# Gwzwpxz/HDSDP

Hardware: AMD Instinct MI355X
Metric: IPM iterations/sec (Schur build+factor+solve), n=2000 m=2000 dense SDP (higher is better)
Workload: dtype f64

## Files before the change

hdsdp_amd/csrc/chol.hip:

```cpp
#include "hdm_common.h"
#include "chol.h"
#include "sweep128.h"
#include <algorithm>
#include <atomic>
#include <cstring>

#define NB 128

#define PB 32
#define LDW 98
__device__ __forceinline__ double hdm_readlane_f64(double v, int lane) {
    int lo = __double2loint(v), hi = __double2hiint(v);
    lo = __builtin_amdgcn_readlane(lo, lane);
    hi = __builtin_amdgcn_readlane(hi, lane);
    return __hiloint2double(hi, lo);
}

typedef double hdm_c4 __attribute__((ext_vector_type(4)));

template <int NT>
__device__ __forceinline__ void hdm_lds_mm(double *pc, int crs, int ccs, const double *pa, int ars, int acs, const double *pb,
                                           int brs, int bcs, int M, int N, int K, double alpha, int accumulate, int k_by_row,
                                           int lower_only, int wave, int lane, double *gout, long gld) {
    const int l15 = lane & 15, lq = lane >> 4;
    const int mt = M >> 4, nt = (N >> 4) / NT, units = mt * nt;
    for (int u = wave; u < units; u += 4) {
        const int ti = u / nt, tj = (u % nt) * NT;
        if (lower_only && tj > ti) continue;
        hdm_c4 acc[NT];
#pragma unroll
        for (int q = 0; q < NT; ++q) acc[q] = (hdm_c4){0.0, 0.0, 0.0, 0.0};
        const int kend = k_by_row ? min(K, (ti + 1) * 16) : K;
        const double *qa = pa + (ti * 16 + l15) * ars + lq * acs;
        const double *qb = pb + lq * brs + (tj * 16 + l15) * bcs;
        for (int k0 = 0; k0 < kend; k0 += 4) {
            const double av = qa[k0 * acs];
#pragma unroll
            for (int q = 0; q < NT; ++q) acc[q] = __builtin_amdgcn_mfma_f64_16x16x4f64(qb[k0 * brs + q * 16 * bcs], av, acc[q], 0, 0, 0);
        }
#pragma unroll
        for (int q = 0; q < NT; ++q)
#pragma unroll
            for (int r = 0; r < 4; ++r) {
                const int m = ti * 16 + l15, n = (tj + q) * 16 + lq + 4 * r;
                double *c = pc + m * crs + n * ccs;
                const double v = (accumulate ? *c : 0.0) + alpha * acc[q][r];
                *c = v;
                if (gout) gout[m + (long) n * gld] = v;
            }
    }
}

__global__ __launch_bounds__(256) void hdm_potrf_diag_kernel(double *__restrict__ A, long ld, double *__restrict__ Dinv,
                                                              int *__restrict__ info, int col0) {
    extern __shared__ __attribute__((aligned(16))) double sm[];
    double *a = sm;
    double *w = sm + NB * NB;
    const int tid = threadIdx.x;
    for (int e0 = tid; e0 < NB * NB; e0 += 256 * 16) {
        double v[16];
#pragma unroll
        for (int q = 0; q < 16; ++q) {
            const int e = e0 + q * 256;
            v[q] = A[(e & (NB - 1)) + (long) (e >> 7) * ld];
        }
#pragma unroll
        for (int q = 0; q < 16; ++q) {
            const int e = e0 + q * 256;
            a[e] = ((e & (NB - 1)) >= (e >> 7)) ? v[q] : 0.0;
        }
    }
    __syncthreads();

    for (int p = 0; p < NB / PB; ++p) {
        const int c0 = p * PB;
        if (tid < 64) {
            const int l = tid & 31;
            double *blk = a + c0 + c0 * NB;
            double row[PB], rinv[PB];
#pragma unroll
            for (int k = 0; k < PB; ++k) row[k] = blk[l + k * NB];
            int bad = 0;
#pragma unroll
            for (int j = 0; j < PB; ++j) {
                double d = hdm_readlane_f64(row[j], j);
                if (!(d > 0.0)) {
                    if (!bad) bad = j + 1;
                    d = 1.0;
                }
                const double piv = sqrt(d);
                double ri = 1.0 / piv;
                asm volatile("" : "+v"(ri));
                rinv[j] = ri;
                row[j] = (l == j) ? piv : row[j] * ri;
#pragma unroll
                for (int k = j + 1; k < PB; ++k) row[k] -= row[j] * hdm_readlane_f64(row[j], k);
                __builtin_amdgcn_sched_barrier(0);
            }
            if (bad && tid == 0) atomicCAS(info, 0, col0 + c0 + bad);
            if (tid < PB) {
#pragma unroll
                for (int k = 0; k < PB; ++k)
                    if (k <= l) A[(c0 + l) + (long) (c0 + k) * ld] = row[k];
            }
#pragma unroll
            for (int k = 0; k < PB; ++k) asm volatile("" : "+v"(row[k]));
            double x[PB];
#pragma unroll
            for (int i = 0; i < PB; ++i) {
                double sacc = (l == i) ? 1.0 : 0.0;
#pragma unroll
                for (int k = 0; k < i; ++k) sacc -= hdm_readlane_f64(row[k], i) * x[k];
                x[i] = (l <= i) ? sacc * rinv[i] : 0.0;
                __builtin_amdgcn_sched_barrier(0);
            }
            if (tid < PB) {
#pragma unroll
                for (int i = 0; i < PB; ++i) blk[i + l * NB] = x[i];
            }
        }
        __syncthreads();
        const int t0 = c0 + PB, nr = NB - t0;
        if (nr <= 0) break;
        const int wave = tid >> 6, lane = tid & 63;
        hdm_lds_mm<2>(a + t0 + c0 * NB, 1, NB, a + t0 + c0 * NB, 1, NB, a + c0 + c0 * NB, NB, 1, nr, PB, PB, 1.0, 0, 0, 0, wave,
                      lane, A + t0 + (long) c0 * ld, ld);
        __syncthreads();
        hdm_lds_mm<1>(a + t0 + t0 * NB, 1, NB, a + t0 + c0 * NB, 1, NB, a + t0 + c0 * NB, NB, 1, nr, nr, PB, -1.0, 1, 0, 1, wave,
                      lane, nullptr, 0);
        __syncthreads();
    }
    {
        const int wave = tid >> 6, lane = tid & 63;
        for (int j = NB / PB - 2; j >= 0; --j) {
            const int c0 = j * PB, r0 = c0 + PB, nr = NB - r0;
            hdm_lds_mm<2>(w, 1, LDW, a + r0 + c0 * NB, 1, NB, a + c0 + c0 * NB, 1, NB, nr, PB, PB, 1.0, 0, 0, 0, wave, lane,
                          nullptr, 0);
            __syncthreads();
            hdm_lds_mm<2>(a + r0 + c0 * NB, 1, NB, a + r0 + r0 * NB, 1, NB, w, 1, LDW, nr, PB, nr, -1.0, 0, 1, 0, wave, lane,
                          nullptr, 0);
            __syncthreads();
        }
    }
    for (int e = tid; e < NB * NB; e += 256) Dinv[e] = a[e];
}

#define DIAG_SWEEP_LDS_DOUBLES (SMALL_P * (SMALL_P + 1) + 2 * SMALL_P)
template <bool SIGNED = false>
__device__ __forceinline__ void hdm_potrf_diag_sweep_body(double *__restrict__ A, long ld, double *__restrict__ Dinv, int *__restrict__ info,
                                                          int col0, int nv, double *__restrict__ sgn_out = nullptr,
                                                          int *__restrict__ nneg_out = nullptr) {
    extern __shared__ __attribute__((aligned(16))) double sm[];
    double *img = sm;
    double *rsv = sm + SMALL_P * (SMALL_P + 1);
    constexpr int ldi = SMALL_P + 1;
    const int tid = threadIdx.x, ty = tid >> 5, tx = tid & 31;
    const int ei = tid & (SMALL_P - 1), ej0 = tid >> 7;
#pragma unroll 8
    for (int j = ej0; j < SMALL_P; j += SM_T / SMALL_P) img[ei + j * ldi] = (ei >= j) ? A[ei + (long) j * ld] : 0.0;
    __syncthreads();
    double a[SM_NR][SM_NC], rr[SM_NR][SM_NC];
#pragma unroll
    for (int r = 0; r < SM_NR; ++r)
#pragma unroll
        for (int c = 0; c < SM_NC; ++c) a[r][c] = img[(ty + 16 * r) + (tx + 32 * c) * ldi];
    __syncthreads();
    double unused;
    int nneg = 0;
    const int bad = sm_sweep<false, SIGNED>(nv, a, rr, img, rsv, ty, tx, &unused, &nneg);
    if (bad && tid == 0) atomicCAS(info, 0, col0 + bad);
    if (SIGNED) {
        if (tid < SMALL_P && sgn_out) sgn_out[tid] = (tid < nv && rsv[tid] < 0.0) ? -1.0 : 1.0;
        if (tid == 0 && nneg_out && nneg) atomicAdd(nneg_out, nneg);
    }
    __syncthreads();
    sm_store_one<true>(SMALL_P, a, img, A, ld, ty, tx, tid);
    sm_store_one<false>(SMALL_P, rr, img, Dinv, SMALL_P, ty, tx, tid);
}
__global__ __launch_bounds__(SM_T) void hdm_potrf_diag_sweep_kernel(double *__restrict__ A, long ld, double *__restrict__ Dinv,
                                                                    int *__restrict__ info, int col0, int nv) {
    hdm_potrf_diag_sweep_body(A, ld, Dinv, info, col0, nv);
}
__global__ __launch_bounds__(SM_T) void hdm_potrf_diag_sweep_signed_kernel(double *__restrict__ A, long ld, double *__restrict__ Dinv,
                                                                           int *__restrict__ info, int col0, int nv,
                                                                           double *__restrict__ sgn) {
    hdm_potrf_diag_sweep_body<true>(A, ld, Dinv, info, col0, nv, sgn, info + 1);
}
template <bool SIGNED>
__global__ __launch_bounds__(SM_T) void hdm_potrf_diag_sweep_tiles_kernel(double *__restrict__ tiles, const int *__restrict__ diag_tile,
                                                                          const int *__restrict__ cols, double *__restrict__ Winv,
                                                                          int *__restrict__ info, int m, double *__restrict__ sgn) {
    const int k = cols[blockIdx.x];
    int dummy = 0;
    (void) dummy;
    double *A = tiles + ((long) diag_tile[k] << 14);
    __shared__ int linfo;
    if (threadIdx.x == 0) linfo = 0;
    __syncthreads();
    hdm_potrf_diag_sweep_body<SIGNED>(A, SMALL_P, Winv + ((long) k << 14), &linfo, k * SMALL_P, min(SMALL_P, m - k * SMALL_P),
                                      SIGNED ? sgn + (long) k * SMALL_P : nullptr, SIGNED ? info + 1 : nullptr);
    __syncthreads();
    if (threadIdx.x == 0 && linfo) {
        int old = atomicCAS(info, 0, linfo);
        while (old != 0 && linfo < old) { const int seen = atomicCAS(info, old, linfo); if (seen == old) break; old = seen; }
    }
}
int hdm_potrf_sweep_configure() {
    HDM_HIP_CHECK(hipFuncSetAttribute((const void *) hdm_potrf_diag_sweep_tiles_kernel<false>, hipFuncAttributeMaxDynamicSharedMemorySize,
                                      DIAG_SWEEP_LDS_DOUBLES * (int) sizeof(double)));
    HDM_HIP_CHECK(hipFuncSetAttribute((const void *) hdm_potrf_diag_sweep_tiles_kernel<true>, hipFuncAttributeMaxDynamicSharedMemorySize,
                                      DIAG_SWEEP_LDS_DOUBLES * (int) sizeof(double)));
    return 0;
}
int hdm_potrf_sweep_batched(double *tiles, const int *diag_tile, const int *cols, int ncols, double *Winv, int *info, int m, hipStream_t s,
                            double *sgn) {
    if (ncols <= 0) return 0;
    if (sgn)
        hipLaunchKernelGGL(hdm_potrf_diag_sweep_tiles_kernel<true>, dim3(ncols), dim3(SM_T), DIAG_SWEEP_LDS_DOUBLES * sizeof(double), s, tiles,
                           diag_tile, cols, Winv, info, m, sgn);
    else
        hipLaunchKernelGGL(hdm_potrf_diag_sweep_tiles_kernel<false>, dim3(ncols), dim3(SM_T), DIAG_SWEEP_LDS_DOUBLES * sizeof(double), s, tiles,
                           diag_tile, cols, Winv, info, m, sgn);
    HDM_HIP_CHECK(hipGetLastError());
    return 0;
}

__global__ void hdm_pad_identity_kernel(double *A, long ld, int n, int npad) {
    long e = (long) blockIdx.x * blockDim.x + threadIdx.x;
    long tot = (long) npad * npad;
    if (e >= tot) return;
    int i = (int) (e % npad), j = (int) (e / npad);
    if (i >= n || j >= n) A[i + (long) j * ld] = (i == j) ? 1.0 : 0.0;
}

__global__ void hdm_reverse_factor_kernel(const double *__restrict__ F, double *__restrict__ W, long ld, int n, int npad) {
    long e = (long) blockIdx.x * blockDim.x + threadIdx.x;
    long tot = (long) npad * npad;
    if (e >= tot) return;
    int i = (int) (e % npad), j = (int) (e / npad);
    double v;
    if (i >= n || j >= n) v = (i == j) ? 1.0 : 0.0;
    else v = (i >= j) ? F[(n - 1 - j) + (long) (n - 1 - i) * ld] : 0.0;
    W[i + (long) j * ld] = v;
}

__global__ void hdm_signed_panel_kernel(double *__restrict__ P, long ld, double *__restrict__ Z, long ldz,
                                        const double *__restrict__ sg, int rows) {
    const long e = (long) blockIdx.x * blockDim.x + threadIdx.x;
    if (e >= (long) rows * NB) return;
    const int i = (int) (e % rows), j = (int) (e / rows);
    const double q = P[i + (long) j * ld];
    Z[i + (long) j * ldz] = q;
    P[i + (long) j * ld] = q * sg[j];
}
__global__ void hdm_reverse_signs_kernel(const double *__restrict__ sgn, double *__restrict__ sig, int n, int npad) {
    const int i = blockIdx.x * blockDim.x + threadIdx.x;
    if (i < npad) sig[i] = (i < n) ? sgn[n - 1 - i] : 1.0;
}
__global__ void hdm_zero_words_kernel(int *p, int count) { if ((int) threadIdx.x < count) p[threadIdx.x] = 0; }

__global__ void hdm_copy_diag_blocks_kernel(const double *__restrict__ Dinv, double *__restrict__ Linv, long ld) {
    const int e = blockIdx.x * 256 + threadIdx.x, k = blockIdx.y;
    Linv[(long) k * NB * (ld + 1) + (e & (NB - 1)) + (long) (e >> 7) * ld] = Dinv[(long) k * NB * NB + e];
}

__global__ void hdm_copy_block_kernel(const double *__restrict__ src, long lds_, double *__restrict__ dst, long ldd,
                                      int rows, int cols) {
    long e = (long) blockIdx.x * blockDim.x + threadIdx.x;
    if (e >= (long) rows * cols) return;
    int i = (int) (e % rows), j = (int) (e / rows);
    dst[i + (long) j * ldd] = src[i + (long) j * lds_];
}

__global__ void hdm_get_diag_kernel(const double *__restrict__ A, long ld, int n, double *__restrict__ d) {
    int i = blockIdx.x * blockDim.x + threadIdx.x;
    if (i < n) d[i] = A[i + (long) i * ld];
}

__global__ __launch_bounds__(256) void hdm_trsv_fwd_step(const double *__restrict__ L, long ld,
                                                          const double *__restrict__ Dinv, double *__restrict__ b,
                                                          double *__restrict__ x, int k, int nblk, int nrhs, long ldv) {
    __shared__ double yk[NB];
    __shared__ double part[256];
    const int tid = threadIdx.x;
    const int bi = k + blockIdx.x;
    const int rhs = blockIdx.y;
    double *bb = b + (long) rhs * ldv, *xx = x + (long) rhs * ldv;
    const double *D = Dinv + (long) k * NB * NB;
    {
        int r = tid & (NB - 1), h = tid >> 7;
        double s = 0.0;
        for (int c = h; c <= r; c += 2) s += D[r + c * NB] * bb[k * NB + c];
        part[tid] = s;
        __syncthreads();
        if (tid < NB) yk[tid] = part[tid] + part[tid + NB];
        __syncthreads();
    }
    if (bi == k) {
        if (tid < NB) xx[k * NB + tid] = yk[tid];
        return;
    }
    if (bi >= nblk) return;
    {
        int r = tid & (NB - 1), h = tid >> 7;
        const double *Lb = L + (long) bi * NB + (long) k * NB * ld;
        double s = 0.0;
        for (int c = h * 64; c < h * 64 + 64; ++c) s += Lb[r + (long) c * ld] * yk[c];
        part[tid] = s;
        __syncthreads();
        if (tid < NB) bb[bi * NB + tid] -= part[tid] + part[tid + NB];
    }
}

__global__ __launch_bounds__(256) void hdm_trsv_bwd_step(const double *__restrict__ L, long ld,
                                                          const double *__restrict__ Dinv, double *__restrict__ y,
                                                          double *__restrict__ x, int k, int nrhs, long ldv) {
    __shared__ double xk[NB];
    __shared__ double part[256];
    const int tid = threadIdx.x;
    const int bi = (int) blockIdx.x;
    const int rhs = blockIdx.y;
    double *yy = y + (long) rhs * ldv, *xx = x + (long) rhs * ldv;
    const double *D = Dinv + (long) k * NB * NB;
    {
        int c = tid & (NB - 1), h = tid >> 7;
        double s = 0.0;
        for (int r = c + h; r < NB; r += 2) s += D[r + c * NB] * yy[k * NB + r];
        part[tid] = s;
        __syncthreads();
        if (tid < NB) xk[tid] = part[tid] + part[tid + NB];
        __syncthreads();
    }
    if (bi == k) {
        if (tid < NB) xx[k * NB + tid] = xk[tid];
        return;
    }
    {
        const double *Lb = L + (long) k * NB + (long) bi * NB * ld;
        const int lane = tid & 63, wave = tid >> 6;
        for (int cc = 0; cc < 32; ++cc) {
            int c = wave * 32 + cc;
            double s = Lb[lane + (long) c * ld] * xk[lane] + Lb[lane + 64 + (long) c * ld] * xk[lane + 64];
            for (int off = 32; off > 0; off >>= 1) s += __shfl_down(s, off, 64);
            if (lane == 0) yy[bi * NB + c] -= s;
        }
    }
}

__device__ __forceinline__ bool hdm_flow_wait(const int *flag, int epoch) {
    for (int it = 0; it < (1 << 22); ++it) {
        if (__hip_atomic_load(flag, __ATOMIC_ACQUIRE, __HIP_MEMORY_SCOPE_AGENT) == epoch) return true;
        __builtin_amdgcn_s_sleep(2);
    }
    return false;
}

__device__ __forceinline__ double hdm_row_dot_half(const double *__restrict__ Mb, long ld, const double *v, int tid) {
    const int r = tid & (NB - 1), h = tid >> 7;
    const double *q = Mb + r + (long) (h * 64) * ld;
    double s0 = 0.0, s1 = 0.0;
#pragma unroll 16
    for (int c = 0; c < 64; c += 2) {
        s0 += q[(long) c * ld] * v[h * 64 + c];
        s1 += q[(long) (c + 1) * ld] * v[h * 64 + c + 1];
    }
    return s0 + s1;
}
template <bool SUBTRACT>
__device__ __forceinline__ void hdm_col_dots(const double *__restrict__ Mb, long ld, const double *v, double *out, int wave,
                                             int lane) {
    const double v0 = v[lane], v1 = v[lane + 64];
    for (int cc = 0; cc < 32; cc += 8) {
        double sacc[8];
#pragma unroll
        for (int q = 0; q < 8; ++q) {
            const double *col = Mb + (long) (wave * 32 + cc + q) * ld;
            sacc[q] = col[lane] * v0 + col[lane + 64] * v1;
        }
#pragma unroll
        for (int off = 32; off > 0; off >>= 1)
#pragma unroll
            for (int q = 0; q < 8; ++q) sacc[q] += __shfl_down(sacc[q], off, 64);
        if (lane == 0) {
#pragma unroll
            for (int q = 0; q < 8; ++q) {
                if (SUBTRACT) out[wave * 32 + cc + q] -= sacc[q];
                else out[wave * 32 + cc + q] = sacc[q];
            }
        }
    }
}

__global__ __launch_bounds__(256) void hdm_trsv_flow_kernel(const double *__restrict__ L, long ld,
                                                             const double *__restrict__ Dinv, const double *b, double *y,
                                                             double *x, int nblk, long ldv, int *flags, int epoch,
                                                             int which, volatile int *err, const int *__restrict__ env) {
    __shared__ double v[NB];
    __shared__ double acc[NB];
    __shared__ double part[256];
    __shared__ int ok;
    const int tid = threadIdx.x, lane = tid & 63, wave = tid >> 6;
    const int i = blockIdx.x, rhs = blockIdx.y;
    const double *bb = b + (long) rhs * ldv;
    double *yy = y + (long) rhs * ldv, *xx = x + (long) rhs * ldv;
    int *ff = flags + (long) rhs * 2 * nblk, *fb = ff + nblk;
    const double *D = Dinv + (long) i * NB * NB;
    if (tid < NB) acc[tid] = bb[i * NB + tid];
    if (tid == 0) ok = 1;
    __syncthreads();
    const int kfirst = env ? env[i] : 0, klast = env ? env[nblk + i] : nblk - 1;
    if (which != 2) {
        for (int k = kfirst; k < i; ++k) {
            if (tid == 0 && !hdm_flow_wait(ff + k, epoch)) ok = 0;
            __syncthreads();
            if (!ok) { if (tid == 0) *err = 1; return; }
            __builtin_amdgcn_fence(__ATOMIC_ACQUIRE, "agent");
            if (tid < NB) v[tid] = __builtin_nontemporal_load(yy + k * NB + tid);
            __syncthreads();
            part[tid] = hdm_row_dot_half(L + (long) i * NB + (long) k * NB * ld, ld, v, tid);
            __syncthreads();
            if (tid < NB) acc[tid] -= part[tid] + part[tid + NB];
            __syncthreads();
        }
        part[tid] = hdm_row_dot_half(D, NB, acc, tid);
        __syncthreads();
        if (tid < NB) {
            const double val = part[tid] + part[tid + NB];
            acc[tid] = val;
            yy[i * NB + tid] = val;
            if (which == 1) xx[i * NB + tid] = val;
        }
        __threadfence();
        __syncthreads();
        if (tid == 0) __hip_atomic_store(ff + i, epoch, __ATOMIC_RELEASE, __HIP_MEMORY_SCOPE_AGENT);
        if (which == 1) return;
    }
    for (int k = klast; k > i; --k) {
        if (tid == 0 && !hdm_flow_wait(fb + k, epoch)) ok = 0;
        __syncthreads();
        if (!ok) { if (tid == 0) *err = 1; return; }
        __builtin_amdgcn_fence(__ATOMIC_ACQUIRE, "agent");
        if (tid < NB) v[tid] = __builtin_nontemporal_load(xx + k * NB + tid);
        __syncthreads();
        hdm_col_dots<true>(L + (long) k * NB + (long) i * NB * ld, ld, v, acc, wave, lane);
        __syncthreads();
    }
    hdm_col_dots<false>(D, NB, acc, part, wave, lane);
    __syncthreads();
    if (tid < NB) xx[i * NB + tid] = part[tid];
    __threadfence();
    __syncthreads();
    if (tid == 0) __hip_atomic_store(fb + i, epoch, __ATOMIC_RELEASE, __HIP_MEMORY_SCOPE_AGENT);
}

__global__ void hdm_probe_spd_block_kernel(double *A, long ld) {
    const int e = blockIdx.x * blockDim.x + threadIdx.x;
    const int i = e & (NB - 1), j = e >> 7;
    if (j < NB) A[i + (long) j * ld] = (i == j) ? 4.0 + 0.01 * i : 1.0 / (1.0 + abs(i - j));
}
double hdm_diag_block_probe(int variant, int reps, hipStream_t s) {
    HdmBuf<double> A_own, D_own;
    HdmBuf<int> info_own;
    hipEvent_t e0, e1;
    if (A_own.alloc(NB * NB) != hipSuccess || D_own.alloc(NB * NB) != hipSuccess ||
        info_own.alloc(1) != hipSuccess || hipEventCreate(&e0) != hipSuccess || hipEventCreate(&e1) != hipSuccess)
        return -1.0;
    double *A = A_own.get(), *D = D_own.get();
    int *info = info_own.get();
    (void) hipFuncSetAttribute((const void *) hdm_potrf_diag_kernel, hipFuncAttributeMaxDynamicSharedMemorySize, (NB * NB + LDW * PB) * (int) sizeof(double));
    (void) hipFuncSetAttribute((const void *) hdm_potrf_diag_sweep_kernel, hipFuncAttributeMaxDynamicSharedMemorySize, DIAG_SWEEP_LDS_DOUBLES * (int) sizeof(double));
    (void) hipMemsetAsync(info, 0, sizeof(int), s);
    float ms = 0.f, total = 0.f;
    for (int r = -2; r < reps; ++r) {
        hipLaunchKernelGGL(hdm_probe_spd_block_kernel, dim3(NB * NB / 256), dim3(256), 0, s, A, (long) NB);
        (void) hipEventRecord(e0, s);
        if (variant)
            hipLaunchKernelGGL(hdm_potrf_diag_sweep_kernel, dim3(1), dim3(SM_T), DIAG_SWEEP_LDS_DOUBLES * sizeof(double), s, A, (long) NB, D, info, 0, NB);
        else
            hipLaunchKernelGGL(hdm_potrf_diag_kernel, dim3(1), dim3(256), (NB * NB + LDW * PB) * sizeof(double), s, A, (long) NB, D, info, 0);
        (void) hipEventRecord(e1, s);
        (void) hipEventSynchronize(e1);
        (void) hipEventElapsedTime(&ms, e0, e1);
        if (r >= 0) total += ms;
    }
    (void) hipEventDestroy(e0); (void) hipEventDestroy(e1);
    return total / reps * 1e3;
}

int HdmChol::init(int n_) {
    n = n_;
    npad = (int) hdm_roundup(n, NB);
    nblk = npad / NB;
    size_t mat = sizeof(double) * (size_t) npad * npad;
    HDM_HIP_CHECK(L.alloc((size_t) npad * npad));
    HDM_HIP_CHECK(Dinv.alloc((size_t) nblk * NB * NB));
    HDM_HIP_CHECK(info_dev.alloc(1));
    HDM_HIP_CHECK(vec.alloc((size_t) npad * 4));
    HDM_HIP_CHECK(hdm_memset_sync(L.get(), 0, mat));
    HDM_HIP_CHECK(hipFuncSetAttribute((const void *) hdm_potrf_diag_kernel, hipFuncAttributeMaxDynamicSharedMemorySize,
                                      (NB * NB + LDW * PB) * (int) sizeof(double)));
    HDM_HIP_CHECK(hipFuncSetAttribute((const void *) hdm_potrf_diag_sweep_kernel, hipFuncAttributeMaxDynamicSharedMemorySize,
                                      DIAG_SWEEP_LDS_DOUBLES * (int) sizeof(double)));
    return 0;
}

int HdmChol::set_envelope(const int *first) {
    env_first.clear(); env_colh.clear();
    env_dev.reset();
    if (factor_graph) { (void) hipGraphExecDestroy(factor_graph); factor_graph = nullptr; factor_runs = 0; }
    if (!first || nblk <= 1) return 0;
    env_first.assign(first, first + nblk);
    env_colh.assign(nblk, 0);
    for (int i = 0; i < nblk; ++i) {
        env_first[i] = std::max(0, std::min(env_first[i], i));
        if (i > 0) env_first[i] = std::min(env_first[i], i);
    }
    for (int k = 0; k < nblk; ++k) env_colh[k] = k;
    for (int i = 0; i < nblk; ++i)
        for (int k = env_first[i]; k <= i; ++k) env_colh[k] = std::max(env_colh[k], i);
    for (int k = 1; k < nblk; ++k) env_colh[k] = std::max(env_colh[k], env_colh[k - 1]);
    std::vector<int> both(env_first);
    both.insert(both.end(), env_colh.begin(), env_colh.end());
    HDM_HIP_CHECK(env_dev.alloc(both.size()));
    HDM_HIP_CHECK(hdm_memcpy_h2d_sync(env_dev.get(), both.data(), sizeof(int) * both.size()));
    return 0;
}

void HdmChol::destroy() {
    if (factor_graph) (void) hipGraphExecDestroy(factor_graph);
    for (int i = 0; i < nsolves; ++i) if (solves[i].exec) (void) hipGraphExecDestroy(solves[i].exec);
    factor_graph = nullptr; nsolves = 0;
}

int HdmChol::load_host(const double *A, long lda, hipStream_t s) {
    HDM_HIP_CHECK(hipMemcpy2DAsync(L.get(), sizeof(double) * npad, A, sizeof(double) * lda, sizeof(double) * n, n,
                                   hipMemcpyHostToDevice, s));
    return finish_load(s);
}

int HdmChol::load_device(const double *A, long lda, hipStream_t s) {
    HDM_HIP_CHECK(hipMemcpy2DAsync(L.get(), sizeof(double) * npad, A, sizeof(double) * lda, sizeof(double) * n, n,
                                   hipMemcpyDeviceToDevice, s));
    return finish_load(s);
}

int HdmChol::finish_load(hipStream_t s) {
    if (npad != n) {
        long tot = (long) npad * npad;
        hipLaunchKernelGGL(hdm_pad_identity_kernel, dim3((unsigned) ((tot + 255) / 256)), dim3(256), 0, s, L.get(),
                           (long) npad, n, npad);
        HDM_HIP_CHECK(hipGetLastError());
    }
    factored = false;
    have_inv = false;
    logdet_ok = false;
    return 0;
}

int HdmChol::set_reverse_inverse(hipStream_t s) {
    if (!factored) return 1;
    HDM_HIP_CHECK(Linv.reserve((size_t) npad * npad));
    long tot = (long) npad * npad;
    hipLaunchKernelGGL(hdm_reverse_factor_kernel, dim3((unsigned) ((tot + 255) / 256)), dim3(256), 0, s, L.get(), Linv.get(),
                       (long) npad, n, npad);
    HDM_HIP_CHECK(hipGetLastError());
    have_inv = true;
    return 0;
}

static int hdm_k128_launch(bool update, const double *A, long lda, const double *B, long ldb, double *C, long ldc, int rows,
                           hipStream_t s);
int HdmChol::factor_signed(hipStream_t s, int *info_host, int *nneg_host) {
    if (!sgn.get()) {
        HDM_HIP_CHECK(sgn.alloc((size_t) npad));
        HDM_HIP_CHECK(sinfo_dev.alloc(2));
        HDM_HIP_CHECK(hipFuncSetAttribute((const void *) hdm_potrf_diag_sweep_signed_kernel, hipFuncAttributeMaxDynamicSharedMemorySize,
                                          DIAG_SWEEP_LDS_DOUBLES * (int) sizeof(double)));
    }
    if (!Z.get() && nblk > 1) HDM_HIP_CHECK(Z.alloc((size_t) npad * NB));
    hipLaunchKernelGGL(hdm_zero_words_kernel, dim3(1), dim3(64), 0, s, sinfo_dev.get(), 2);
    HDM_HIP_CHECK(hipGetLastError());
    const long ld = npad;
    static const bool k128 = [] { const char *e = getenv("HDM_CHOL_K128"); return !(e && atoi(e) == 0); }();
    for (int k = 0; k < nblk; ++k) {
        double *Akk = L.get() + (long) k * NB * (ld + 1);
        hipLaunchKernelGGL(hdm_potrf_diag_sweep_signed_kernel, dim3(1), dim3(SM_T), DIAG_SWEEP_LDS_DOUBLES * sizeof(double), s, Akk, ld,
                           Dinv.get() + (long) k * NB * NB, sinfo_dev.get(), k * NB, std::max(1, std::min(NB, n - k * NB)), sgn.get() + (long) k * NB);
        HDM_HIP_CHECK(hipGetLastError());
        const int rows = npad - (k + 1) * NB;
        if (rows <= 0) break;
        double *P = Akk + NB;
        if (k128 && rows % 64 == 0 && ld < (1L << 20)) {
            if (hdm_k128_launch(false, P, ld, Dinv.get() + (long) k * NB * NB, NB, P, ld, rows, s)) return 1;
        } else {
            HdmGemmArgs g = {};
            g.A = P; g.lda = ld; g.B = Dinv.get() + (long) k * NB * NB; g.ldb = NB; g.C = P; g.ldc = ld;
            g.M = rows; g.N = NB; g.K = NB; g.batch = 1; g.alpha = 1.0; g.beta = 0.0; g.epilogue = HDM_EPI_STORE;
            if (hdm_launch_gemm(g, s)) return 1;
        }
        const long tot = (long) rows * NB;
        hipLaunchKernelGGL(hdm_signed_panel_kernel, dim3((unsigned) ((tot + 255) / 256)), dim3(256), 0, s, P, ld, Z.get(), (long) npad,
                           (const double *) (sgn.get() + (long) k * NB), rows);
        HDM_HIP_CHECK(hipGetLastError());
        if (k128 && rows % 64 == 0 && ld < (1L << 20)) {
            if (hdm_k128_launch(true, P, ld, Z.get(), (long) npad, Akk + (long) NB * (ld + 1), ld, rows, s)) return 1;
        } else {
            HdmGemmArgs u = {};
            u.A = P; u.lda = ld; u.B = Z.get(); u.ldb = npad; u.C = Akk + (long) NB * (ld + 1); u.ldc = ld;
            u.M = rows; u.N = rows; u.K = NB; u.batch = 1; u.alpha = -1.0; u.beta = 1.0;
            u.lower_only = 1; u.epilogue = HDM_EPI_STORE;
            if (hdm_launch_gemm(u, s)) return 1;
        }
    }
    int info[2] = {0, 0};
    HDM_HIP_CHECK(hipMemcpyAsync(info, sinfo_dev.get(), sizeof(int) * 2, hipMemcpyDeviceToHost, s));
    HDM_HIP_CHECK(hipStreamSynchronize(s));
    if (info[0] > n) info[0] = 0;
    if (info_host) *info_host = info[0];
    if (nneg_host) *nneg_host = info[1];
    factored = (info[0] == 0);
    have_inv = false;
    logdet_ok = false;
    return 0;
}

int HdmChol::reverse_signs(double *sig_dev, hipStream_t s) {
    if (!sgn.get() || !factored) return 1;
    hipLaunchKernelGGL(hdm_reverse_signs_kernel, dim3((npad + 255) / 256), dim3(256), 0, s, (const double *) sgn.get(), sig_dev, n, npad);
    HDM_HIP_CHECK(hipGetLastError());
    return 0;
}

template <class F> static hipGraphExec_t hdm_capture(hipStream_t s, F body) {
    hipGraph_t graph = nullptr;
    hipGraphExec_t exec = nullptr;
    if (hipStreamBeginCapture(s, hipStreamCaptureModeThreadLocal) != hipSuccess) { (void) hipGetLastError(); return nullptr; }
    hdm_gemm_capture_mode(1);
    const int rc = body();
    hdm_gemm_capture_mode(0);
    const hipError_t e = hipStreamEndCapture(s, &graph);
    if (rc || e != hipSuccess || !graph) { (void) hipGetLastError(); if (graph) (void) hipGraphDestroy(graph); return nullptr; }
    if (hipGraphInstantiate(&exec, graph, nullptr, nullptr, 0) != hipSuccess) { (void) hipGetLastError(); exec = nullptr; }
    (void) hipGraphDestroy(graph);
    return exec;
}
static int hdm_graph_level() {
    static int lvl = -1;
    if (lvl < 0) { const char *e = getenv("HDM_GRAPHS"); lvl = e ? atoi(e) : 0; }
    return lvl;
}

int HdmChol::factor(hipStream_t s, int *info_host) {
    if (hdm_graph_level() >= 1 && nblk >= 4 && graphs_ok && !factor_graph && factor_runs >= 1) {
        factor_graph = hdm_capture(s, [&]() { return enqueue_factor(s); });
        if (!factor_graph) graphs_ok = false;
    }
    if (factor_graph) HDM_HIP_CHECK(hipGraphLaunch(factor_graph, s));
    else if (enqueue_factor(s)) return 1;
    ++factor_runs;
    int info = 0;
    HDM_HIP_CHECK(hipMemcpyAsync(&info, info_dev.get(), sizeof(int), hipMemcpyDeviceToHost, s));
    HDM_HIP_CHECK(hipStreamSynchronize(s));
    if (info > n) info = 0;
    if (info_host) *info_host = info;
    factored = (info == 0);
    have_inv = false;
    return 0;
}

typedef unsigned hdm_k2 __attribute__((ext_vector_type(2)));
template <int NJ, bool UPDATE>
__global__ __launch_bounds__(256) void hdm_k128_kernel(const double *__restrict__ A, long lda, const double *__restrict__ B, long ldb,
                                                       double *C, long ldc) {
    constexpr int KB = (NJ == 2) ? 8 : 4;
    const int ti = blockIdx.x, tj = blockIdx.y;
    if (UPDATE && ti < tj) return;
    const int tid = threadIdx.x, lane = tid & 63;
    const int wave = __builtin_amdgcn_readfirstlane(tid >> 6);
    const int l15 = lane & 15, lq = lane >> 4;
    const int r0 = ti * 64 + (wave & 1) * 32, c0 = tj * (32 * NJ) + (wave >> 1) * (16 * NJ);
    const __amdgpu_buffer_rsrc_t ra = __builtin_amdgcn_make_buffer_rsrc(const_cast<double *>(A + r0), 0, 0x7fffffff, 0x00020000);
    const __amdgpu_buffer_rsrc_t rb = __builtin_amdgcn_make_buffer_rsrc(const_cast<double *>(B + c0), 0, 0x7fffffff, 0x00020000);
    const unsigned va = (unsigned) ((l15 + lq * lda) * 8), vb = (unsigned) ((l15 + lq * ldb) * 8);
    const unsigned sa = (unsigned) (4 * lda * 8), sb = (unsigned) (4 * ldb * 8);
    hdm_c4 acc[NJ][2];
#pragma unroll
    for (int j = 0; j < NJ; ++j)
#pragma unroll
        for (int i = 0; i < 2; ++i) acc[j][i] = (hdm_c4){0.0, 0.0, 0.0, 0.0};
    hdm_k2 fa[2][KB][NJ], fb[2][KB][2];
#define K128_LOAD(SET, BLK)                                                                                      \
    _Pragma("unroll") for (int q = 0; q < KB; ++q) {                                                             \
        _Pragma("unroll") for (int i = 0; i < 2; ++i)                                                            \
            fb[SET][q][i] = __builtin_amdgcn_raw_buffer_load_b64(ra, va + 128 * i, ((BLK) * KB + q) * sa, 0);    \
        _Pragma("unroll") for (int j = 0; j < NJ; ++j)                                                           \
            fa[SET][q][j] = __builtin_amdgcn_raw_buffer_load_b64(rb, vb + 128 * j, ((BLK) * KB + q) * sb, 0);    \
    }
#define K128_MMA(SET)                                                                                            \
    _Pragma("unroll") for (int q = 0; q < KB; ++q)                                                               \
        _Pragma("unroll") for (int j = 0; j < NJ; ++j)                                                           \
            _Pragma("unroll") for (int i = 0; i < 2; ++i)                                                        \
                acc[j][i] = __builtin_amdgcn_mfma_f64_16x16x4f64(__builtin_bit_cast(double, fa[SET][q][j]),      \
                                                                 __builtin_bit_cast(double, fb[SET][q][i]), acc[j][i], 0, 0, 0);
    constexpr int NBLK = 32 / KB;
    K128_LOAD(0, 0) K128_LOAD(1, 1)
#pragma unroll
    for (int b = 0; b < NBLK; b += 2) {
        K128_MMA(0)
        if (b + 2 < NBLK) { K128_LOAD(0, b + 2) }
        K128_MMA(1)
        if (b + 3 < NBLK) { K128_LOAD(1, b + 3) }
    }
#undef K128_LOAD
#undef K128_MMA
    if (!UPDATE) __syncthreads();
    double *cl = C + (r0 + l15) + (long) (c0 + lq) * ldc;
    const bool diag = UPDATE && (ti == tj);
#pragma unroll
    for (int j = 0; j < NJ; ++j)
#pragma unroll
        for (int r = 0; r < 4; ++r)
#pragma unroll
            for (int i = 0; i < 2; ++i) {
                double *q = cl + 16 * i + (long) (16 * j + 4 * r) * ldc;
                if (UPDATE) {
                    if (diag && (r0 + 16 * i + l15) < (c0 + 16 * j + lq + 4 * r)) continue;
                    *q = -1.0 * acc[j][i][r] + 1.0 * (*q);
                } else {
                    *q = 1.0 * acc[j][i][r];
                }
            }
}

static int hdm_k128_launch(bool update, const double *A, long lda, const double *B, long ldb, double *C, long ldc, int rows,
                           hipStream_t s) {
    if (update) hipLaunchKernelGGL((hdm_k128_kernel<2, true>), dim3(rows / 64, rows / 64), dim3(256), 0, s, A, lda, B, ldb, C, ldc);
    else hipLaunchKernelGGL((hdm_k128_kernel<4, false>), dim3(rows / 64, 1), dim3(256), 0, s, A, lda, B, ldb, C, ldc);
    HDM_HIP_CHECK(hipGetLastError());
    return 0;
}

__global__ void hdm_zero_word_kernel(int *p) { *p = 0; }

int HdmChol::enqueue_factor(hipStream_t s) {
    hipLaunchKernelGGL(hdm_zero_word_kernel, dim3(1), dim3(1), 0, s, info_dev.get());
    HDM_HIP_CHECK(hipGetLastError());
    const long ld = npad;
    const size_t shm = (NB * NB + LDW * PB) * sizeof(double);
    static const bool diag_sweep = [] { const char *e = getenv("HDM_DIAG_SWEEP"); return !(e && atoi(e) == 0); }();
    for (int k = 0; k < nblk; ++k) {
        double *Akk = L.get() + (long) k * NB * (ld + 1);
        if (diag_sweep)
            hipLaunchKernelGGL(hdm_potrf_diag_sweep_kernel, dim3(1), dim3(SM_T), DIAG_SWEEP_LDS_DOUBLES * sizeof(double), s, Akk, ld,
                               Dinv.get() + (long) k * NB * NB, info_dev.get(), k * NB, std::max(1, std::min(NB, n - k * NB)));
        else
            hipLaunchKernelGGL(hdm_potrf_diag_kernel, dim3(1), dim3(256), shm, s, Akk, ld, Dinv.get() + (long) k * NB * NB,
                               info_dev.get(), k * NB);
        HDM_HIP_CHECK(hipGetLastError());
        if (npad - (k + 1) * NB <= 0) break;
        const int rows = env_colh.empty() ? npad - (k + 1) * NB : (env_colh[k] - k) * NB;
        if (rows <= 0) continue;
        double *P = Akk + NB;
        static const bool k128 = [] { const char *e = getenv("HDM_CHOL_K128"); return !(e && atoi(e) == 0); }();
        if (k128 && rows % 64 == 0 && ld < (1L << 20)) {
            if (hdm_k128_launch(false, P, ld, Dinv.get() + (long) k * NB * NB, NB, P, ld, rows, s)) return 1;
            if (hdm_k128_launch(true, P, ld, P, ld, Akk + (long) NB * (ld + 1), ld, rows, s)) return 1;
            continue;
        }
        HdmGemmArgs g = {};
        g.A = P; g.lda = ld; g.B = Dinv.get() + (long) k * NB * NB; g.ldb = NB; g.C = P; g.ldc = ld;
        g.M = rows; g.N = NB; g.K = NB; g.batch = 1; g.alpha = 1.0; g.beta = 0.0;
        g.epilogue = HDM_EPI_STORE;
        if (hdm_launch_gemm(g, s)) return 1;
        HdmGemmArgs u = {};
        u.A = P; u.lda = ld; u.B = P; u.ldb = ld; u.C = Akk + (long) NB * (ld + 1); u.ldc = ld;
        u.M = rows; u.N = rows; u.K = NB; u.batch = 1; u.alpha = -1.0; u.beta = 1.0;
        u.lower_only = 1; u.epilogue = HDM_EPI_STORE;
        if (hdm_launch_gemm(u, s)) return 1;
    }
    return 0;
}

int HdmChol::invert_factor(hipStream_t s) {
    if (have_inv) return 0;
    const long ld = npad;
    size_t mat = sizeof(double) * (size_t) npad * npad;
    HDM_HIP_CHECK(Linv.reserve(mat / sizeof(double)));
    if (!Z.get() && nblk > 1) HDM_HIP_CHECK(Z.alloc((size_t) npad * NB));
    HDM_HIP_CHECK(hipMemsetAsync(Linv.get(), 0, mat, s));
    if (nblk >= 2 && (nblk & (nblk - 1)) == 0) {
        HDM_HIP_CHECK(Zd.reserve(mat / sizeof(double)));
        hipLaunchKernelGGL(hdm_copy_diag_blocks_kernel, dim3(NB * NB / 256, nblk), dim3(256), 0, s, Dinv.get(), Linv.get(), ld);
        HDM_HIP_CHECK(hipGetLastError());
        for (long sz = NB; sz < npad; sz *= 2) {
            const int pairs = (int) (npad / (2 * sz));
            const long pstride = 2 * sz * (ld + 1);
            HdmGemmArgs g = {};
            g.A = L.get() + sz; g.lda = ld; g.strideA = pstride;
            g.B = Linv.get(); g.ldb = ld; g.b_kmajor = 1; g.strideB = pstride;
            g.C = Zd.get() + sz; g.ldc = ld; g.strideC = pstride;
            g.M = (int) sz; g.N = (int) sz; g.K = (int) sz; g.batch = pairs; g.alpha = 1.0; g.epilogue = HDM_EPI_STORE;
            if (hdm_launch_gemm(g, s)) return 1;
            HdmGemmArgs h = {};
            h.A = Linv.get() + sz * (ld + 1); h.lda = ld; h.strideA = pstride;
            h.B = Zd.get() + sz; h.ldb = ld; h.b_kmajor = 1; h.strideB = pstride;
            h.C = Linv.get() + sz; h.ldc = ld; h.strideC = pstride;
            h.M = (int) sz; h.N = (int) sz; h.K = (int) sz; h.batch = pairs; h.alpha = -1.0;
            h.klimit = HDM_KLIM_BY_M; h.epilogue = HDM_EPI_STORE;
            if (hdm_launch_gemm(h, s)) return 1;
        }
        have_inv = true;
        return 0;
    }
    for (int k = nblk - 1; k >= 0; --k) {
        double *Xkk = Linv.get() + (long) k * NB * (ld + 1);
        hipLaunchKernelGGL(hdm_copy_block_kernel, dim3(NB * NB / 256), dim3(256), 0, s, Dinv.get() + (long) k * NB * NB,
                           (long) NB, Xkk, ld, NB, NB);
        HDM_HIP_CHECK(hipGetLastError());
        const int rows = npad - (k + 1) * NB;
        if (rows <= 0) continue;
        const double *P = L.get() + (long) k * NB * (ld + 1) + NB;
        HdmGemmArgs g = {};
        g.A = P; g.lda = ld; g.B = Dinv.get() + (long) k * NB * NB; g.ldb = NB; g.b_kmajor = 1;
        g.C = Z.get(); g.ldc = npad; g.M = rows; g.N = NB; g.K = NB; g.batch = 1; g.alpha = 1.0; g.epilogue = HDM_EPI_STORE;
        if (hdm_launch_gemm(g, s)) return 1;
        HdmGemmArgs h = {};
        h.A = Linv.get() + (long) (k + 1) * NB * (ld + 1); h.lda = ld; h.B = Z.get(); h.ldb = npad; h.b_kmajor = 1;
        h.C = Xkk + NB; h.ldc = ld; h.M = rows; h.N = NB; h.K = rows; h.batch = 1; h.alpha = -1.0;
        h.klimit = HDM_KLIM_BY_M; h.epilogue = HDM_EPI_STORE;
        if (hdm_launch_gemm(h, s)) return 1;
    }
    have_inv = true;
    return 0;
}

int HdmChol::get_diag(double *diag_host, hipStream_t s) {
    hipLaunchKernelGGL(hdm_get_diag_kernel, dim3((n + 255) / 256), dim3(256), 0, s, L.get(), (long) npad, n, vec.get());
    HDM_HIP_CHECK(hipGetLastError());
    HDM_HIP_CHECK(hipMemcpyAsync(diag_host, vec.get(), sizeof(double) * n, hipMemcpyDeviceToHost, s));
    HDM_HIP_CHECK(hipStreamSynchronize(s));
    return 0;
}

static std::atomic<int> g_flow_shared_device{0};
void hdm_flow_set_shared_device(int on) { g_flow_shared_device.store(on); }
bool hdm_flow_shared_device() { return g_flow_shared_device.load() != 0; }
static bool hdm_flow_enabled() {
    static int on = -1;
    if (on < 0) { const char *e = getenv("HDM_TRSV_FLOW"); on = (e && atoi(e) == 0) ? 0 : 1; }
    return on == 1 && g_flow_shared_device.load() == 0;
}

int HdmChol::solve_device(double *b_dev, double *x_dev, int nrhs, long ldv, int which, hipStream_t s) {
    if (hdm_graph_level() >= 2 && graphs_ok && !(hdm_flow_enabled() && flow_ok)) {
        Replay *r = nullptr;
        for (int i = 0; i < nsolves; ++i)
            if (solves[i].b == b_dev && solves[i].x == x_dev && solves[i].nrhs == nrhs && solves[i].which == which &&
                solves[i].ldv == ldv) r = &solves[i];
        if (!r && solve_runs >= 1 && nsolves < 4) {
            hipGraphExec_t ex = hdm_capture(s, [&]() { return enqueue_solve(b_dev, x_dev, nrhs, ldv, which, s); });
            if (!ex) graphs_ok = false;
            else { r = &solves[nsolves++]; r->b = b_dev; r->x = x_dev; r->nrhs = nrhs; r->which = which; r->ldv = ldv; r->exec = ex; }
        }
        if (r) {
            HDM_HIP_CHECK(hipGraphLaunch(r->exec, s));
            return 0;
        }
    }
    ++solve_runs;
    return enqueue_solve(b_dev, x_dev, nrhs, ldv, which, s);
}

int HdmChol::enqueue_solve(double *b_dev, double *x_dev, int nrhs, long ldv, int which, hipStream_t s) {
    const long ld = npad;
    if (flow_cap < 0) {
        int dev = 0, cus = 0, per_cu = 0;
        if (hipGetDevice(&dev) == hipSuccess &&
            hipDeviceGetAttribute(&cus, hipDeviceAttributeMultiprocessorCount, dev) == hipSuccess &&
            hipOccupancyMaxActiveBlocksPerMultiprocessor(&per_cu, hdm_trsv_flow_kernel, 256, 0) == hipSuccess)
            flow_cap = cus * std::max(1, per_cu);
        else
            flow_cap = 0;
        (void) hipGetLastError();
    }
    if (hdm_flow_enabled() && flow_ok && nrhs <= 2 && (long) nblk * nrhs <= flow_cap) {
        if (!flow_flags) {
            HDM_HIP_CHECK(flow_flags.alloc(4 * (size_t) nblk));
            HDM_HIP_CHECK(hdm_memset_sync(flow_flags.get(), 0, sizeof(int) * 4 * (size_t) nblk));
            HDM_HIP_CHECK(flow_err.alloc(1, hipHostMallocMapped));
            *flow_err.get() = 0;
        }
        int *err_dev = flow_err.dev();
        ++flow_epoch;
        hipLaunchKernelGGL(hdm_trsv_flow_kernel, dim3(nblk, nrhs), dim3(256), 0, s, L.get(), ld, Dinv.get(), b_dev, b_dev, x_dev, nblk,
                           ldv, flow_flags.get(), flow_epoch, which, err_dev, (const int *) env_dev.get());
        HDM_HIP_CHECK(hipGetLastError());
        flow_pending = true;
        return 0;
    }
    double *cur = b_dev;
    if (which == 0 || which == 1) {
        for (int k = 0; k < nblk; ++k) {
            hipLaunchKernelGGL(hdm_trsv_fwd_step, dim3(nblk - k, nrhs), dim3(256), 0, s, L.get(), ld, Dinv.get(), cur, x_dev, k,
                               nblk, nrhs, ldv);
        }
        HDM_HIP_CHECK(hipGetLastError());
        if (which == 1) return 0;
        HDM_HIP_CHECK(hipMemcpyAsync(cur, x_dev, sizeof(double) * ldv * nrhs, hipMemcpyDeviceToDevice, s));
    }
    for (int k = nblk - 1; k >= 0; --k) {
        hipLaunchKernelGGL(hdm_trsv_bwd_step, dim3(k + 1, nrhs), dim3(256), 0, s, L.get(), ld, Dinv.get(), cur, x_dev, k, nrhs,
                           ldv);
    }
    HDM_HIP_CHECK(hipGetLastError());
    return 0;
}

static bool hdm_flow_fail_once() {
    static int left = -1;
    if (left < 0) { const char *e = getenv("HDM_TRSV_FLOW_FAIL_ONCE"); left = (e && atoi(e) != 0) ? 1 : 0; }
    if (left == 1) { left = 0; return true; }
    return false;
}

int HdmChol::solve_host(const double *rhs, double *sol, int nrhs, int which, hipStream_t s) {
    const int chunk = 2;
    if (host_stage.size() < (size_t) chunk * n) host_stage.resize((size_t) chunk * n);
    for (int c0 = 0; c0 < nrhs; c0 += chunk) {
        int nc = (nrhs - c0 < chunk) ? nrhs - c0 : chunk;
        double *b = vec.get(), *x = vec.get() + 2L * npad;
        HDM_HIP_CHECK(hipMemsetAsync(vec.get(), 0, sizeof(double) * 4L * npad, s));
        HDM_HIP_CHECK(hipMemcpy2DAsync(b, sizeof(double) * npad, rhs + (long) c0 * n, sizeof(double) * n,
                                       sizeof(double) * n, nc, hipMemcpyHostToDevice, s));
        if (solve_device(b, x, nc, npad, which, s)) return 1;
        HDM_HIP_CHECK(hipMemcpy2DAsync(host_stage.data(), sizeof(double) * n, x, sizeof(double) * npad,
                                       sizeof(double) * n, nc, hipMemcpyDeviceToHost, s));
        HDM_HIP_CHECK(hipStreamSynchronize(s));
        bool gave_up = flow_pending && flow_err && *(volatile int *) flow_err.get() != 0;
        if (flow_pending && hdm_flow_fail_once()) gave_up = true;
        flow_pending = false;
        if (gave_up) {
            fprintf(stderr, "[hdsdp_mi355x] single-launch substitution timed out; using per-block launches\n");
            flow_ok = false;
            if (flow_err) *flow_err.get() = 0;
            c0 -= chunk;
            continue;
        }
        memcpy(sol + (long) c0 * n, host_stage.data(), sizeof(double) * (size_t) n * nc);
    }
    return 0;
}

int HdmChol::inverse_full(double *out_dev, long ldo, hipStream_t s) {
    if (invert_factor(s)) return 1;
    HdmGemmArgs g = {};
    g.A = Linv.get(); g.lda = npad; g.a_kmajor = 1; g.B = Linv.get(); g.ldb = npad; g.b_kmajor = 1;
    g.C = out_dev; g.ldc = ldo; g.M = npad; g.N = npad; g.K = npad; g.batch = 1; g.alpha = 1.0;
    g.epilogue = HDM_EPI_STORE;
    return hdm_launch_gemm(g, s);
}

const void *hdm_module_handle_chol() { return (const void *) hdm_potrf_diag_kernel; }
```

Measured before the change: 2.861.

## Add MFMA-based diagonal-block Cholesky kernel and make it default

Adds a new single-workgroup kernel that factors each 128x128 diagonal block and builds its inverse factor (Dinv) using f64 MFMA 16x16x4 matrix instructions on panels held in LDS. Wave 0 factors each 32-column panel with register sweeps while the other waves load the block, apply trailing and triangular-inverse updates, and write Dinv. It becomes the default diagonal path, targeting the serial per-block latency on the critical path of the blocked factorization. The older sweep kernel remains selectable through an environment variable. The risks are more complex synchronisation and numerical ordering, plus occupancy pressure from the large LDS footprint.

```diff
diff --git a/hdsdp_amd/csrc/chol.hip b/hdsdp_amd/csrc/chol.hip
--- a/hdsdp_amd/csrc/chol.hip
+++ b/hdsdp_amd/csrc/chol.hip
@@ -223,6 +223,229 @@
                            diag_tile, cols, Winv, info, m, sgn);
     HDM_HIP_CHECK(hipGetLastError());
     return 0;
+}
+
+#define DLD 129
+#define DIAG_MFMA_LDS_DOUBLES (NB * DLD)
+__device__ __forceinline__ void hdm_pin(double &v) { asm volatile("" : "+v"(v)); }
+__device__ __forceinline__ void hdm_tri_decode(int t, int &ti, int &tj) {
+    ti = 0;
+    while ((ti + 1) * (ti + 2) / 2 <= t) ++ti;
+    tj = t - ti * (ti + 1) / 2;
+}
+template <int NT, int KS>
+__device__ __forceinline__ void hdm_blk_mm(double *pc, int crs, int ccs, const double *pa, int ars, int acs, const double *pb,
+                                           int brs, int bcs, int nt, double alpha, bool accumulate, bool lower, int ubeg, int uend,
+                                           int w, int nw, int lane, double *gout, long gld) {
+    const int l15 = lane & 15, lq = lane >> 4;
+    for (int u = ubeg + w; u < uend; u += 2 * nw) {
+        const bool two = u + nw < uend;
+        int ti[2], tj[2];
+#pragma unroll
+        for (int h = 0; h < 2; ++h) {
+            const int uu = (h == 1 && two) ? u + nw : u;
+            if (lower) hdm_tri_decode(uu, ti[h], tj[h]);
+            else { ti[h] = uu / nt; tj[h] = (uu % nt) * NT; }
+        }
+        double av[2][KS], bv[2][KS][NT], cv[2][NT][4];
+        hdm_c4 acc[2][NT];
+#pragma unroll
+        for (int h = 0; h < 2; ++h) {
+            const double *qa = pa + (ti[h] * 16 + l15) * ars + lq * acs;
+            const double *qb = pb + lq * brs + (tj[h] * 16 + l15) * bcs;
+#pragma unroll
+            for (int s = 0; s < KS; ++s) {
+                av[h][s] = qa[4 * s * acs];
+#pragma unroll
+                for (int q = 0; q < NT; ++q) bv[h][s][q] = qb[4 * s * brs + q * 16 * bcs];
+            }
+#pragma unroll
+            for (int q = 0; q < NT; ++q)
+#pragma unroll
+                for (int r = 0; r < 4; ++r)
+                    cv[h][q][r] = accumulate ? pc[(ti[h] * 16 + l15) * crs + ((tj[h] + q) * 16 + lq + 4 * r) * ccs] : 0.0;
+        }
+#pragma unroll
+        for (int h = 0; h < 2; ++h)
+#pragma unroll
+            for (int q = 0; q < NT; ++q) acc[h][q] = (hdm_c4){0.0, 0.0, 0.0, 0.0};
+#pragma unroll
+        for (int s = 0; s < KS; ++s)
+#pragma unroll
+            for (int h = 0; h < 2; ++h)
+#pragma unroll
+                for (int q = 0; q < NT; ++q) acc[h][q] = __builtin_amdgcn_mfma_f64_16x16x4f64(bv[h][s][q], av[h][s], acc[h][q], 0, 0, 0);
+#pragma unroll
+        for (int h = 0; h < 2; ++h) {
+            if (h == 1 && !two) break;
+#pragma unroll
+            for (int q = 0; q < NT; ++q)
+#pragma unroll
+                for (int r = 0; r < 4; ++r) {
+                    const int m = ti[h] * 16 + l15, n = (tj[h] + q) * 16 + lq + 4 * r;
+                    const double v = cv[h][q][r] + alpha * acc[h][q][r];
+                    pc[m * crs + n * ccs] = v;
+                    if (gout) gout[m + (long) n * gld] = v;
+                }
+        }
+    }
+}
+template <int NT>
+__device__ __forceinline__ void hdm_blk_mm_tri(double *pc, int crs, int ccs, const double *pa, int ars, int acs, const double *pb,
+                                               int brs, int bcs, int nt, int units, int K, int w, int nw, int lane) {
+    const int l15 = lane & 15, lq = lane >> 4;
+    for (int u = w; u < units; u += nw) {
+        const int ti = u / nt, tj = (u % nt) * NT;
+        hdm_c4 acc[NT];
+#pragma unroll
+        for (int q = 0; q < NT; ++q) acc[q] = (hdm_c4){0.0, 0.0, 0.0, 0.0};
+        const double *qa = pa + (ti * 16 + l15) * ars + lq * acs;
+        const double *qb = pb + lq * brs + (tj * 16 + l15) * bcs;
+        for (int k0 = tj * 16; k0 < K; k0 += 16) {
+            double av[4], bv[4][NT];
+#pragma unroll
+            for (int s = 0; s < 4; ++s) {
+                av[s] = qa[(k0 + 4 * s) * acs];
+#pragma unroll
+                for (int q = 0; q < NT; ++q) bv[s][q] = qb[(k0 + 4 * s) * brs + q * 16 * bcs];
+            }
+#pragma unroll
+            for (int s = 0; s < 4; ++s)
+#pragma unroll
+                for (int q = 0; q < NT; ++q) acc[q] = __builtin_amdgcn_mfma_f64_16x16x4f64(bv[s][q], av[s], acc[q], 0, 0, 0);
+        }
+#pragma unroll
+        for (int q = 0; q < NT; ++q)
+#pragma unroll
+            for (int r = 0; r < 4; ++r) pc[(ti * 16 + l15) * crs + ((tj + q) * 16 + lq + 4 * r) * ccs] = acc[q][r];
+    }
+}
+
+__global__ __launch_bounds__(256) void hdm_potrf_diag_mfma_kernel(double *__restrict__ A, long ld, double *__restrict__ Dinv,
+                                                                   int *__restrict__ info, int col0, int nv) {
+    extern __shared__ __attribute__((aligned(16))) double sm[];
+    double *a = sm;
+    double *tsc = a + 96 * DLD;
+    double *stash = a + 32 * DLD;
+    const int tid = threadIdx.x, lane = tid & 63;
+    const int wave = __builtin_amdgcn_readfirstlane(tid >> 6);
+    const int mlive = min(NB, (nv + 15) & ~15);
+    const int nsub = (min(nv, NB) + PB - 1) / PB;
+    for (int p = 0; p < nsub; ++p) {
+        const int c0 = p * PB;
+        double *blk = a + c0 + c0 * DLD;
+        const int mt = (mlive - c0) >> 4, ntot = mt * (mt + 1) / 2;
+        if (wave == 0) {
+            const int l = lane & 31;
+            const bool upper = lane >= 32;
+            double row[PB];
+            if (p == 0) {
+#pragma unroll
+                for (int k = 0; k < PB; ++k) row[k] = A[l + (long) k * ld];
+#pragma unroll
+                for (int k = 0; k < PB; ++k) {
+                    hdm_pin(row[k]);
+                    row[k] = upper ? ((k == l) ? 1.0 : 0.0) : (l >= k && l < nv) ? row[k] : (k == l) ? 1.0 : 0.0;
+                }
+            } else {
+                hdm_blk_mm<1, PB / 4>(blk, 1, DLD, blk - PB * DLD, 1, DLD, blk - PB * DLD, DLD, 1, 1, -1.0, true, true, 0, min(3, ntot), 0, 1,
+                                      lane, nullptr, 0);
+#pragma unroll
+                for (int k = 0; k < PB; ++k) row[k] = blk[l + k * DLD];
+#pragma unroll
+                for (int k = 0; k < PB; ++k) {
+                    hdm_pin(row[k]);
+                    row[k] = upper ? ((k == l) ? 1.0 : 0.0) : row[k];
+                }
+            }
+            int bad = 0;
+#pragma unroll
+            for (int j = 0; j < PB; ++j) {
+                double d = hdm_readlane_f64(row[j], j);
+                const bool neg = !(d > 0.0);
+                bad = (neg && bad == 0) ? j + 1 : bad;
+                d = neg ? 1.0 : d;
+                const double rs = sm_rsqrt(d);
+                row[j] *= rs;
+#pragma unroll
+                for (int k = j + 1; k < PB; ++k) row[k] -= row[j] * hdm_readlane_f64(row[j], k);
+            }
+            if (bad && lane == 0) atomicCAS(info, 0, col0 + c0 + bad);
+            double *dst = upper ? blk + l * DLD : stash + l;
+            const int dstr = upper ? 1 : DLD;
+#pragma unroll
+            for (int k = 0; k < PB; ++k) dst[k * dstr] = row[k];
+        } else if (p == 0) {
+            for (int jb = wave - 1; jb < NB; jb += 45) {
+                double v0[15], v1[15];
+#pragma unroll
+                for (int q = 0; q < 15; ++q) {
+                    const int j = min(jb + 3 * q, NB - 1);
+                    v0[q] = A[lane + (long) j * ld];
+                    v1[q] = A[lane + 64 + (long) j * ld];
+                }
+#pragma unroll
+                for (int q = 0; q < 15; ++q) {
+                    const int j = jb + 3 * q, i0 = lane, i1 = lane + 64;
+                    hdm_pin(v0[q]);
+                    hdm_pin(v1[q]);
+                    if (j < NB) {
+                        if (!(i0 < PB && j < 2 * PB)) a[i0 + j * DLD] = (i0 >= j && i0 < nv) ? v0[q] : (i0 == j) ? 1.0 : 0.0;
+                        a[i1 + j * DLD] = (i1 >= j && i1 < nv) ? v1[q] : (i1 == j) ? 1.0 : 0.0;
+                    }
+                }
+            }
+        } else {
+            hdm_blk_mm<1, PB / 4>(blk, 1, DLD, blk - PB * DLD, 1, DLD, blk - PB * DLD, DLD, 1, 1, -1.0, true, true, 3, ntot, wave - 1, 3,
+                                  lane, nullptr, 0);
+            hdm_blk_mm_tri<2>(tsc, DLD, 1, a + c0, 1, DLD, a, 1, DLD, p, 2 * p, c0, wave - 1, 3, lane);
+            if (p == 3) {
+                const int t = tid - 64, i = t % 96;
+                for (int j0 = t / 96; j0 < NB; j0 += 32) {
+                    double v[16];
+#pragma unroll
+                    for (int q = 0; q < 16; ++q) v[q] = a[i + (j0 + 2 * q) * DLD];
+#pragma unroll
+                    for (int q = 0; q < 16; ++q) {
+                        hdm_pin(v[q]);
+                        Dinv[i + (j0 + 2 * q) * NB] = (i >= j0 + 2 * q) ? v[q] : 0.0;
+                    }
+                }
+            }
+        }
+        __syncthreads();
+        {
+            const int i = tid & (PB - 1), j0 = tid >> 5;
+            double v[4];
+#pragma unroll
+            for (int q = 0; q < 4; ++q) v[q] = stash[i + (j0 + 8 * q) * DLD];
+#pragma unroll
+            for (int q = 0; q < 4; ++q) {
+                hdm_pin(v[q]);
+                if (i >= j0 + 8 * q) A[(c0 + i) + (long) (c0 + j0 + 8 * q) * ld] = v[q];
+            }
+        }
+        const int t0 = c0 + PB, nr = max(0, mlive - t0);
+        hdm_blk_mm<2, PB / 4>(a + t0 + c0 * DLD, 1, DLD, a + t0 + c0 * DLD, 1, DLD, blk, DLD, 1, 1, 1.0, false, false, 0, nr >> 4, 3 - wave, 4,
+                              lane, A + t0 + (long) c0 * ld, ld);
+        hdm_blk_mm<2, PB / 4>(a + c0, 1, DLD, blk, 1, DLD, tsc, DLD, 1, p, -1.0, false, false, 0, 2 * p, 3 - wave, 4, lane, nullptr, 0);
+        __syncthreads();
+    }
+    const int sh = (nsub == 4) ? 5 : 7, r0 = NB - (1 << sh);
+    for (int e0 = tid; e0 < (NB << sh); e0 += 256 * 16) {
+        double v[16];
+#pragma unroll
+        for (int q = 0; q < 16; ++q) {
+            const int e = e0 + 256 * q;
+            v[q] = a[r0 + (e & ((1 << sh) - 1)) + (e >> sh) * DLD];
+        }
+#pragma unroll
+        for (int q = 0; q < 16; ++q) {
+            const int e = e0 + 256 * q, i = r0 + (e & ((1 << sh) - 1)), j = e >> sh;
+            hdm_pin(v[q]);
+            Dinv[i + j * NB] = (i >= j) ? v[q] : 0.0;
+        }
+    }
 }
 
 __global__ void hdm_pad_identity_kernel(double *A, long ld, int n, int npad) {
@@ -469,12 +692,15 @@
     int *info = info_own.get();
     (void) hipFuncSetAttribute((const void *) hdm_potrf_diag_kernel, hipFuncAttributeMaxDynamicSharedMemorySize, (NB * NB + LDW * PB) * (int) sizeof(double));
     (void) hipFuncSetAttribute((const void *) hdm_potrf_diag_sweep_kernel, hipFuncAttributeMaxDynamicSharedMemorySize, DIAG_SWEEP_LDS_DOUBLES * (int) sizeof(double));
+    (void) hipFuncSetAttribute((const void *) hdm_potrf_diag_mfma_kernel, hipFuncAttributeMaxDynamicSharedMemorySize, DIAG_MFMA_LDS_DOUBLES * (int) sizeof(double));
     (void) hipMemsetAsync(info, 0, sizeof(int), s);
     float ms = 0.f, total = 0.f;
     for (int r = -2; r < reps; ++r) {
         hipLaunchKernelGGL(hdm_probe_spd_block_kernel, dim3(NB * NB / 256), dim3(256), 0, s, A, (long) NB);
         (void) hipEventRecord(e0, s);
-        if (variant)
+        if (variant == 2)
+            hipLaunchKernelGGL(hdm_potrf_diag_mfma_kernel, dim3(1), dim3(256), DIAG_MFMA_LDS_DOUBLES * sizeof(double), s, A, (long) NB, D, info, 0, NB);
+        else if (variant)
             hipLaunchKernelGGL(hdm_potrf_diag_sweep_kernel, dim3(1), dim3(SM_T), DIAG_SWEEP_LDS_DOUBLES * sizeof(double), s, A, (long) NB, D, info, 0, NB);
         else
             hipLaunchKernelGGL(hdm_potrf_diag_kernel, dim3(1), dim3(256), (NB * NB + LDW * PB) * sizeof(double), s, A, (long) NB, D, info, 0);
@@ -501,6 +727,8 @@
                                       (NB * NB + LDW * PB) * (int) sizeof(double)));
     HDM_HIP_CHECK(hipFuncSetAttribute((const void *) hdm_potrf_diag_sweep_kernel, hipFuncAttributeMaxDynamicSharedMemorySize,
                                       DIAG_SWEEP_LDS_DOUBLES * (int) sizeof(double)));
+    HDM_HIP_CHECK(hipFuncSetAttribute((const void *) hdm_potrf_diag_mfma_kernel, hipFuncAttributeMaxDynamicSharedMemorySize,
+                                      DIAG_MFMA_LDS_DOUBLES * (int) sizeof(double)));
     return 0;
 }
 
@@ -747,10 +975,13 @@
     HDM_HIP_CHECK(hipGetLastError());
     const long ld = npad;
     const size_t shm = (NB * NB + LDW * PB) * sizeof(double);
-    static const bool diag_sweep = [] { const char *e = getenv("HDM_DIAG_SWEEP"); return !(e && atoi(e) == 0); }();
+    static const int diag_sweep = [] { const char *e = getenv("HDM_DIAG_SWEEP"); const int v = e ? atoi(e) : 2; return (v == 0 || v == 1) ? v : 2; }();
     for (int k = 0; k < nblk; ++k) {
         double *Akk = L.get() + (long) k * NB * (ld + 1);
-        if (diag_sweep)
+        if (diag_sweep == 2)
+            hipLaunchKernelGGL(hdm_potrf_diag_mfma_kernel, dim3(1), dim3(256), DIAG_MFMA_LDS_DOUBLES * sizeof(double), s, Akk, ld,
+                               Dinv.get() + (long) k * NB * NB, info_dev.get(), k * NB, std::max(1, std::min(NB, n - k * NB)));
+        else if (diag_sweep)
             hipLaunchKernelGGL(hdm_potrf_diag_sweep_kernel, dim3(1), dim3(SM_T), DIAG_SWEEP_LDS_DOUBLES * sizeof(double), s, Akk, ld,
                                Dinv.get() + (long) k * NB * NB, info_dev.get(), k * NB, std::max(1, std::min(NB, n - k * NB)));
         else
```

Result: no change. 2.869 (median of 6 runs) (+0.2%).
